# Leqr/MSMP-PDE

Hardware: AMD Instinct MI355X
Metric: rollout-steps/sec (whole node), E2 nx=100 tw=25 (higher is better)
Workload: dtype f32; 1 GPU; E2 MSMP-PDE (MP_PDE_SolverLEMLinGated), 2048 graphs x nx=100, time_window=25, 6 gated layer pairs, radius graph n=3; graphs_total=2048, graphs_per_gpu=2048, nodes_per_gpu=204800, edges_per_gpu=1204224, parallelism=dp1 (graph-sharded, no collective in the rollout), sub_batches=1, range_policy_switched_to_exact_fp32=False, preheat=170 untimed steps (>= 1 s) after the 5 warm-up steps

## Files before the change

### msmp-pde_amd/csrc/lem_kernel.hip

```cpp
#include "lem_layout.h"
#include <type_traits>

namespace msmp {

struct LemPackArgs {
    const float *w, *wz, *b, *bz, *wa, *ba, *wb, *bb;
    int ninp;
    float* out;
};

__global__ void pack_lem_kernel(LemPackArgs a) {
    const LemLayout L = lem_layout();
    const int kin = H + a.ninp;
    for (int64_t p = (int64_t)blockIdx.x * blockDim.x + threadIdx.x; p < L.scales; p += (int64_t)gridDim.x * blockDim.x) {
        float v = 0.f;
        if (p < L.mlp) {
            const int ch = (int)(p / CHUNK_FLOATS), row = (int)(p % CHUNK_FLOATS) / KC, kk = (int)(p % KC);
            const int grp = ch >> 2, k = (ch & 3) * KC + kk;
            if (grp == 0) v = a.w[(size_t)(H + row) * kin + k];
            else if (grp == 1) v = a.w[(size_t)(2 * H + row) * kin + k];
            else if (grp == 2) v = a.w[(size_t)row * kin + k];
            else v = a.wz[(size_t)row * kin + k];
        } else if (p < L.bias) {
            const int64_t o = p - L.mlp;
// ... 158 lines not shown
        for (int T = 0; T < 4; ++T)
#pragma unroll
            for (int r = 0; r < 16; ++r)
                z[T][0][r] = (1.0f - g[T][0][r]) * z[T][0][r] + g[T][0][r] * tanhf_(acc[T][0][r]);
        lem_acc_init<NS>(a, 0, lane, hh, x, g);
        LEM_GROUP(y, g, 8, a.rec + 12 * CHUNK_FLOATS)
#pragma unroll
        for (int T = 0; T < 4; ++T)
#pragma unroll
            for (int r = 0; r < 16; ++r) g[T][0][r] = a.dt * sigmoidf_(g[T][0][r]);
        lem_acc_init<NS>(a, 3, lane, hh, x, acc);
        LEM_GROUP(z, acc, 12, after)
#pragma unroll
        for (int T = 0; T < 4; ++T)
#pragma unroll
            for (int r = 0; r < 16; ++r)
                y[T][0][r] = (1.0f - g[T][0][r]) * y[T][0][r] + g[T][0][r] * tanhf_(acc[T][0][r]);
    }
#undef LEM_GROUP

    if (a.with_mlp) {
        acc_init_bias<1>(a.mlpb, hh, acc);
#pragma unroll
        for (int j = 0; j < 4; ++j) {
            wstage_load(ws, a.mlp + (size_t)(j + 1) * CHUNK_FLOATS, tid);
            mma_chunk_from_acc<1>(lds + (j & 1) * H * LDW, c, hh, y[j], acc);
            wstage_store(ws, lds + ((j + 1) & 1) * H * LDW, tid);
            __syncthreads();
        }
#pragma unroll
        for (int T = 0; T < 4; ++T)
#pragma unroll
            for (int r = 0; r < 16; ++r) acc[T][0][r] = swishf(acc[T][0][r]);
        acc_init_bias<1>(a.mlpb + H, hh, y);
#pragma unroll
        for (int j = 0; j < 4; ++j) {
            if (j < 3) wstage_load(ws, a.mlp + (size_t)(4 + j + 1) * CHUNK_FLOATS, tid);
            mma_chunk_from_acc<1>(lds + (j & 1) * H * LDW, c, hh, acc[j], y);
            if (j < 3) {
                wstage_store(ws, lds + ((j + 1) & 1) * H * LDW, tid);
                __syncthreads();
            }
        }
#pragma unroll
        for (int T = 0; T < 4; ++T)
#pragma unroll
            for (int r = 0; r < 16; ++r) y[T][0][r] = swishf(y[T][0][r]);
    }

    if (n < a.n_nodes) {
        float* o = a.out + (size_t)n * H + 4 * hh;
#pragma unroll
        for (int T = 0; T < 4; ++T)
#pragma unroll
            for (int q = 0; q < 4; ++q) {
                f32x4 v;
#pragma unroll
                for (int m = 0; m < 4; ++m) v[m] = y[T][0][4 * q + m];
                *reinterpret_cast<f32x4*>(o + 32 * T + 8 * q) = v;
            }
    }
}


struct LemWsArgs {
    const float* xin;
    const float* u;
    const float* pos_x;
    const float* pos_t;
    const float* vars;
    const float* dt_cum;
    int tw, nv;
    long n_nodes;
    int t_len, with_mlp;
    float dt;
    const float* rec_s;
    const float* mlp_s;
    const float* bias_s;
    const float* wx_h;
    const float* mlpb_s;
    const float* scales;
    float* out;
    int full_wgs = 0x7fffffff;
};

constexpr int LEM_WS_FR = 1024;

template <int P, int MODE>
__device__ __forceinline__ void lem_ws_load_x(const LemWsArgs& a, const float* xc, long node, int t, float (&x)[2 * ((P + 1) / 2)]) {
    constexpr int NS = (P + 1) / 2;
    if (MODE == 0) {
        const f32x2* p = reinterpret_cast<const f32x2*>(a.xin + ((size_t)node * a.t_len + t) * (2 * NS));
#pragma unroll
        for (int i = 0; i < NS; ++i) {
            const f32x2 v = p[i];
            x[2 * i] = v[0];
            x[2 * i + 1] = v[1];
        }
    } else {
#pragma unroll
        for (int i = 0; i < NS; ++i) {
            const f32x2 v = *reinterpret_cast<const f32x2*>(xc + 2 * i);
            x[2 * i] = v[0];
            x[2 * i + 1] = v[1];
        }
        if (MODE == 1) {
            x[1] = a.u[(size_t)node * a.tw + t];
        } else {
            x[1] = a.u[(size_t)node * 2 * a.tw + t];
            x[2] = a.u[(size_t)node * 2 * a.tw + a.tw + t];
            x[3] = a.dt_cum[t] + x[3];
        }
    }
}

template <int P>
__device__ __forceinline__ void lem_ws_slots(const float (&x)[2 * ((P + 1) / 2)], int hh, half8 (&bx)[(3 * P + 2 + 15) / 16]) {
    constexpr int M = (3 * P + 2 + 15) / 16;
    _Float16 xh[P], xl[P];
#pragma unroll
    for (int f = 0; f < P; ++f) {
        xh[f] = (_Float16)x[f];
        xl[f] = (_Float16)(x[f] - (float)xh[f]);
    }
#pragma unroll
    for (int m = 0; m < M; ++m)
#pragma unroll
        for (int j = 0; j < 8; ++j) {
            const int s0 = 16 * m + j, s1 = 16 * m + 8 + j;
            const _Float16 v0 = s0 < 3 * P ? (s0 / P == 1 ? xl[s0 % P] : xh[s0 % P]) : (_Float16)(s0 < 3 * P + 2 ? 1.f : 0.f);
            const _Float16 v1 = s1 < 3 * P ? (s1 / P == 1 ? xl[s1 % P] : xh[s1 % P]) : (_Float16)(s1 < 3 * P + 2 ? 1.f : 0.f);
            bx[m][j] = hh ? v1 : v0;
        }
}

template <int P, int MODE>
__device__ __forceinline__ void lem_ws3_patch(const float (&xd)[MODE == 1 ? 1 : 3], int hh, half8 (&bx)[(3 * P + 2 + 15) / 16]) {
    constexpr int ND = MODE == 1 ? 1 : 3;
#pragma unroll
    for (int k = 0; k < ND; ++k) {
        const int f = 1 + k;
        const _Float16 h = (_Float16)xd[k];
        const _Float16 l = (_Float16)(xd[k] - (float)h);
#pragma unroll
        for (int p = 0; p < 3; ++p) {
            const int s = p * P + f, m = s >> 4, hhs = (s >> 3) & 1, j = s & 7;
            bx[m][j] = hh == hhs ? (p == 1 ? l : h) : bx[m][j];
        }
    }
}

__device__ __forceinline__ void lem_ws_bias(const float* bl, int hh, f32x16& acc) {
#pragma unroll
    for (int q = 0; q < 4; ++q) {
        const f32x4 bv = *reinterpret_cast<const f32x4*>(bl + 8 * q + 4 * hh);
#pragma unroll
        for (int m = 0; m < 4; ++m) acc[4 * q + m] = bv[m];
    }
}

__device__ __forceinline__ void lem_ws_publish(const f32x16& st, half8* area, int ks, int lane) {
#pragma unroll
    for (int s = 0; s < 2; ++s) {
        float v[8];
#pragma unroll
        for (int j = 0; j < 8; ++j) v[j] = st[8 * s + j];
        half8 hi, lo;
        split8(v, hi, lo);
        area[((ks * 2 + s) * 2 + 0) * 64 + lane] = hi;
        area[((ks * 2 + s) * 2 + 1) * 64 + lane] = lo;
    }
}

__device__ __forceinline__ float vmin(float a, float b) {
    float d;
    asm("v_min_f32 %0, %1, %2" : "=v"(d) : "v"(a), "v"(b));
    return d;
}

__device__ __forceinline__ void lem_ws_update_publish_q(const f32x16& a0, const f32x16& a1, float c0, float c1, float idt, f32x16& st,
                                                        half8* area, int ks, int lane) {
#pragma unroll
    for (int s = 0; s < 2; ++s) {
        half8 phi, plo;
#pragma unroll
        for (int i = 0; i < 8; i += 2) {
            f32x2 sv;
#pragma unroll
            for (int e = 0; e < 2; ++e) {
                const int r = 8 * s + i + e;
                const float ea = msmp_exp2(a0[r] * c0);
                const float eb = msmp_exp2(vmin(a1[r] * c1, 60.f));
                const float qb = eb + 1.0f;
                const float rr = msmp_rcp(__builtin_fmaf(ea, idt, idt) * qb);
                sv[e] = __builtin_fmaf(rr, __builtin_fmaf(-st[r], qb, 1.0f - eb), st[r]);
                st[r] = sv[e];
            }
            const half2 hp = __builtin_convertvector(sv, half2);
            const half2 lp = split_lo_pair(hp, sv);
            phi[i] = hp[0];
            phi[i + 1] = hp[1];
            plo[i] = lp[0];
            plo[i + 1] = lp[1];
        }
        area[((ks * 2 + s) * 2 + 0) * 64 + lane] = phi;
        area[((ks * 2 + s) * 2 + 1) * 64 + lane] = plo;
    }
}

constexpr int LEM_SCHED_NOT_MFMA = 0x7F6;

#if MSMP_PROF_LEM
__device__ unsigned long long g_prof_lem[16];
#define LPROF_DECL unsigned lp_m = 0, lp_v = 0, lp_b = 0, lp_w = 0, lp_t = (unsigned)__builtin_readcyclecounter();
#define LPROF(var) do { const unsigned t_ = (unsigned)__builtin_readcyclecounter(); var += t_ - lp_t; lp_t = t_; } while (0)
#define LPROF_FLUSH if (lane == 0 && ks == 0 && (blockIdx.x & 31) == 0) { unsigned long long* o = g_prof_lem + 4 * role; atomicAdd(o, (unsigned long long)lp_m); atomicAdd(o + 1, (unsigned long long)lp_v); atomicAdd(o + 2, (unsigned long long)lp_b); atomicAdd(o + 3, 1ull); atomicAdd(g_prof_lem + 8 + role, (unsigned long long)lp_w); }
#else
#define LPROF_DECL unsigned lp_w = 0; (void)lp_w;
#define LPROF(var)
#define LPROF_FLUSH
#endif
#define LEM_SYNC() do { LPROF(lp_w); __syncthreads(); LPROF(lp_b); } while (0)

template <bool SAME, int OFF0, int OFF1>
__device__ __forceinline__ void lem_ws3_gemm2(const half8 (&w0)[4][2][2], const half8 (&w1)[4][2][2], const char* b0, const char* b1,
                                              f32x16& acc0, f32x16& acc1) {
    if (!SAME) {
        constexpr int FB = 64 * 16;
        auto frag = [&](int n, int plane) -> half8 {
            const int f = (n >> 1) * 2 + plane;
            return (n & 1) ? *reinterpret_cast<const half8*>(b1 + OFF1 + f * FB) : *reinterpret_cast<const half8*>(b0 + OFF0 + f * FB);
        };
        half8 h = frag(0, 0), l = frag(0, 1);
#pragma unroll
        for (int n = 0; n < 16; ++n) {
            const int kt = n >> 2, s = (n >> 1) & 1;
            half8 hn = h, ln = l;
            if (n < 15) hn = frag(n + 1, 0);
            __builtin_amdgcn_sched_barrier(0);
            if (n & 1) {
                acc1 = __builtin_amdgcn_mfma_f32_32x32x16_f16(w1[kt][s][1], h, acc1, 0, 0, 0);
                acc1 = __builtin_amdgcn_mfma_f32_32x32x16_f16(w1[kt][s][0], l, acc1, 0, 0, 0);
            } else {
                acc0 = __builtin_amdgcn_mfma_f32_32x32x16_f16(w0[kt][s][1], h, acc0, 0, 0, 0);
                acc0 = __builtin_amdgcn_mfma_f32_32x32x16_f16(w0[kt][s][0], l, acc0, 0, 0, 0);
            }
            __builtin_amdgcn_sched_barrier(0);
            if (n < 15) ln = frag(n + 1, 1);
            __builtin_amdgcn_sched_barrier(0);
            if (n & 1) acc1 = __builtin_amdgcn_mfma_f32_32x32x16_f16(w1[kt][s][0], h, acc1, 0, 0, 0);
            else acc0 = __builtin_amdgcn_mfma_f32_32x32x16_f16(w0[kt][s][0], h, acc0, 0, 0, 0);
            __builtin_amdgcn_sched_barrier(0);
            h = hn;
            l = ln;
        }
        return;
    }
#pragma unroll
    for (int kt = 0; kt < 4; ++kt)
#pragma unroll
        for (int s = 0; s < 2; ++s) {
            constexpr int FB = 64 * 16;
            const int f = (kt * 2 + s) * 2;
            const half8 h0 = *reinterpret_cast<const half8*>(b0 + OFF0 + f * FB), l0 = *reinterpret_cast<const half8*>(b0 + OFF0 + (f + 1) * FB);
            half8 h1 = h0, l1 = l0;
            if (!SAME) {
                h1 = *reinterpret_cast<const half8*>(b1 + OFF1 + f * FB);
                l1 = *reinterpret_cast<const half8*>(b1 + OFF1 + (f + 1) * FB);
            }
            MSMP_MFMA_LOLO(2, acc0, w0[kt][s][1], l0);
            MSMP_MFMA_LOLO(2, acc1, w1[kt][s][1], l1);
            acc0 = __builtin_amdgcn_mfma_f32_32x32x16_f16(w0[kt][s][1], h0, acc0, 0, 0, 0);
            acc0 = __builtin_amdgcn_mfma_f32_32x32x16_f16(w0[kt][s][0], l0, acc0, 0, 0, 0);
            acc0 = __builtin_amdgcn_mfma_f32_32x32x16_f16(w0[kt][s][0], h0, acc0, 0, 0, 0);
            __builtin_amdgcn_sched_barrier(LEM_SCHED_NOT_MFMA);
            acc1 = __builtin_amdgcn_mfma_f32_32x32x16_f16(w1[kt][s][1], h1, acc1, 0, 0, 0);
            acc1 = __builtin_amdgcn_mfma_f32_32x32x16_f16(w1[kt][s][0], l1, acc1, 0, 0, 0);
            acc1 = __builtin_amdgcn_mfma_f32_32x32x16_f16(w1[kt][s][0], h1, acc1, 0, 0, 0);
            __builtin_amdgcn_sched_barrier(LEM_SCHED_NOT_MFMA);
        }
}

template <int P, int MODE>
__global__ __launch_bounds__(512) void lem_encoder_ws3_kernel(LemWsArgs a) {
    constexpr int NS = (P + 1) / 2, M = (3 * P + 2 + 15) / 16;
    __shared__ __attribute__((aligned(16))) float lds[6 * SPLIT_CHUNK_FLOATS + 768];
    __shared__ __attribute__((aligned(16))) float xconst[96 * 8];
    __shared__ half8 bxc[3 * M * 64];
    __shared__ half8 wxl[8 * 2 * M * 64];
    half8* const yfr = reinterpret_cast<half8*>(lds);
    half8* const zfr = yfr + 3 * LEM_WS_FR;
    float* const bias_l = lds + 6 * SPLIT_CHUNK_FLOATS;
    const int tid = threadIdx.x, lane = tid & 63;
    const int wave = __builtin_amdgcn_readfirstlane(tid >> 6);
    const int ks = wave & 3, role = wave >> 2;
    const int c = lane & 31, hh = lane >> 5;
    const bool single = (int)blockIdx.x >= a.full_wgs;
    const long n0 = single ? 96L * a.full_wgs + 32L * ((int)blockIdx.x - a.full_wgs) : (long)blockIdx.x * 96;
    const long n_lim = single ? (n0 + 32 < a.n_nodes ? n0 + 32 : a.n_nodes) : a.n_nodes;
    const int nt = single ? 1 : 3;
    const float LOG2E = 1.44269504088896340736f;
    const float inv_w = a.scales[4], inv_z = a.scales[5];
    const int T = a.t_len;

    {
        half8 zero;
#pragma unroll
        for (int j = 0; j < 8; ++j) zero[j] = (_Float16)0.f;
#pragma unroll
        for (int i = 0; i < 6; ++i) yfr[tid + 512 * i] = zero;
        bias_l[tid] = a.bias_s[tid];
        if (tid < 256) bias_l[512 + tid] = a.mlpb_s[tid];
        if (MODE != 0 && tid < 96) {
            const long nn = n0 + tid < a.n_nodes ? n0 + tid : a.n_nodes - 1;
            float* row = xconst + 8 * tid;
#pragma unroll
            for (int f = 0; f < 8; ++f) row[f] = 0.f;
            row[0] = a.pos_x[nn];
            if (MODE == 1) {
                for (int f = 0; f < a.nv; ++f) row[2 + f] = a.vars[(size_t)nn * a.nv + f];
            } else {
                row[3] = a.pos_t[nn];
                for (int f = 1; f < a.nv; ++f) row[3 + f] = a.vars[(size_t)nn * a.nv + f];
            }
        }
    }
    half8 w[2][4][2][2];
    half8* const wxw = wxl + (size_t)wave * (2 * M * 64) + lane;
    {
        const half8* rs = reinterpret_cast<const half8*>(a.rec_s);
        const half8* wh = reinterpret_cast<const half8*>(a.wx_h);
#pragma unroll
        for (int gi = 0; gi < 2; ++gi) {
            const int grp = 2 * role + gi;
#pragma unroll
            for (int kt = 0; kt < 4; ++kt)
#pragma unroll
                for (int s = 0; s < 2; ++s)
#pragma unroll
                    for (int pl = 0; pl < 2; ++pl)
                        w[gi][kt][s][pl] = rs[(size_t)(grp * 4 + kt) * 1024 + ((s * 4 + ks) * 2 + pl) * 64 + lane];
#pragma unroll
            for (int m = 0; m < M; ++m) wxw[(gi * M + m) * 64] = wh[((grp * 4 + ks) * 2 + m) * 64 + lane];
        }
    }
    const float c0 = -inv_w * LOG2E, c1 = -2.0f * (role ? inv_z : inv_w) * LOG2E, idt = 1.0f / a.dt;

    f32x16 st[3];
#pragma unroll
    for (int X = 0; X < 3; ++X)
#pragma unroll
        for (int r = 0; r < 16; ++r) st[X][r] = 0.f;
    constexpr int ZBASE = 3 * LEM_WS_FR * 16;
    const char* lb_y;
    const char* lb_z;
    {
        unsigned lo = lane * 16;
        asm volatile("" : "+v"(lo));
        lb_y = reinterpret_cast<const char*>(lds) + lo;
        unsigned lo2 = lane * 16 + ZBASE;
        asm volatile("" : "+v"(lo2));
        lb_z = reinterpret_cast<const char*>(lds) + lo2;
    }
    float xn[2 * NS];
    f32x16 acc0, acc1;
#pragma unroll
    for (int r = 0; r < 16; ++r) { acc0[r] = 0.f; acc1[r] = 0.f; }
    __syncthreads();

    float xd[MODE == 1 ? 1 : 3];
    if (MODE != 0 && tid < 192) {
        const int Xt = tid >> 6, l64 = tid & 63;
        float xs[2 * NS];
#pragma unroll
        for (int f = 0; f < 2 * NS; ++f) xs[f] = xconst[8 * (32 * Xt + (l64 & 31)) + f];
        if (MODE == 2) xs[3] = 0.f;
        half8 b0[M];
        lem_ws_slots<P>(xs, l64 >> 5, b0);
#pragma unroll
        for (int m = 0; m < M; ++m) bxc[(Xt * M + m) * 64 + l64] = b0[m];
    }
    __syncthreads();
    auto fetch_x = [&](auto Xc, int t) {
        constexpr int X = decltype(Xc)::value;
        const long n = n0 + 32 * X + c;
        if (MODE != 0) {
            const long node = n < a.n_nodes ? n : a.n_nodes - 1;
            if (MODE == 1) {
                xd[0] = a.u[(size_t)node * a.tw + t];
            } else {
                xd[0] = a.u[(size_t)node * 2 * a.tw + t];
                xd[MODE == 1 ? 0 : 1] = a.u[(size_t)node * 2 * a.tw + a.tw + t];
                xd[MODE == 1 ? 0 : 2] = a.dt_cum[t] + xconst[8 * (32 * X + c) + 3];
            }
            return;
        }
        lem_ws_load_x<P, MODE>(a, xconst + 8 * (32 * X + c), n < a.n_nodes ? n : a.n_nodes - 1, t, xn);
    };
    auto half_m = [&](auto Xc) {
        constexpr int X = decltype(Xc)::value;
        half8 bx[M];
        __builtin_amdgcn_sched_barrier(0);
        if (MODE != 0) {
#pragma unroll
            for (int m = 0; m < M; ++m) bx[m] = bxc[(X * M + m) * 64 + lane];
            lem_ws3_patch<P, MODE>(xd, hh, bx);
        } else {
            lem_ws_slots<P>(xn, hh, bx);
        }
        const f32x16 zero = {0.f, 0.f, 0.f, 0.f, 0.f, 0.f, 0.f, 0.f, 0.f, 0.f, 0.f, 0.f, 0.f, 0.f, 0.f, 0.f};
        acc0 = __builtin_amdgcn_mfma_f32_32x32x16_f16(wxw[0], bx[0], zero, 0, 0, 0);
        acc1 = __builtin_amdgcn_mfma_f32_32x32x16_f16(wxw[M * 64], bx[0], zero, 0, 0, 0);
#pragma unroll
        for (int m = 1; m < M; ++m) {
            acc0 = __builtin_amdgcn_mfma_f32_32x32x16_f16(wxw[m * 64], bx[m], acc0, 0, 0, 0);
            acc1 = __builtin_amdgcn_mfma_f32_32x32x16_f16(wxw[(M + m) * 64], bx[m], acc1, 0, 0, 0);
        }
        constexpr int YO = X * LEM_WS_FR * 16, ZO = (3 + X) * LEM_WS_FR * 16 - ZBASE;
        if (role) lem_ws3_gemm2<false, YO, ZO>(w[0], w[1], lb_y, lb_z, acc0, acc1);
        else lem_ws3_gemm2<true, YO, YO>(w[0], w[1], lb_y, lb_y, acc0, acc1);
    };
    auto half_v = [&](auto Xc) {
        constexpr int X = decltype(Xc)::value;
        lem_ws_update_publish_q(acc0, acc1, c0, c1, idt, st[X], (role ? yfr : zfr) + X * LEM_WS_FR, ks, lane);
    };
    using I0 = std::integral_constant<int, 0>;
    using I1 = std::integral_constant<int, 1>;
    using I2 = std::integral_constant<int, 2>;

    LPROF_DECL
    if (single) {
        if (!role) {
            fetch_x(I0{}, 0);
            for (int t = 0; t < T; ++t) {
                { half_m(I0{}); LPROF(lp_m); }                                                   LEM_SYNC();
                fetch_x(I0{}, t + 1 < T ? t + 1 : t); { half_v(I0{}); LPROF(lp_v); }             LEM_SYNC();
                LEM_SYNC();
                LEM_SYNC();
            }
        } else {
            for (int t = 0; t < T; ++t) {
                LEM_SYNC();
                fetch_x(I0{}, t);                                                               LEM_SYNC();
                { half_m(I0{}); LPROF(lp_m); }                                                   LEM_SYNC();
                { half_v(I0{}); LPROF(lp_v); }                                                   LEM_SYNC();
            }
        }
    } else
    if (!role) {
        fetch_x(I0{}, 0);
        for (int t = 0; t < T; ++t) {
            { half_m(I0{}); LPROF(lp_m); }                                           LEM_SYNC();
            fetch_x(I1{}, t); { half_v(I0{}); LPROF(lp_v); }                         LEM_SYNC();
            { half_m(I1{}); LPROF(lp_m); }                                           LEM_SYNC();
            fetch_x(I2{}, t); { half_v(I1{}); LPROF(lp_v); }                         LEM_SYNC();
            { half_m(I2{}); LPROF(lp_m); }                                           LEM_SYNC();
            fetch_x(I0{}, t + 1 < T ? t + 1 : t); { half_v(I2{}); LPROF(lp_v); }     LEM_SYNC();
        }
        LEM_SYNC();
        LEM_SYNC();
        LEM_SYNC();
    } else {
        LEM_SYNC();
        LEM_SYNC();
        fetch_x(I0{}, 0);                                           LEM_SYNC();
        { half_m(I0{}); LPROF(lp_m); }                                               LEM_SYNC();
        fetch_x(I1{}, 0); { half_v(I0{}); LPROF(lp_v); }                             LEM_SYNC();
        { half_m(I1{}); LPROF(lp_m); }                                               LEM_SYNC();
        for (int t = 1; t < T; ++t) {
            fetch_x(I2{}, t - 1); { half_v(I1{}); LPROF(lp_v); }                     LEM_SYNC();
            { half_m(I2{}); LPROF(lp_m); }                                           LEM_SYNC();
            fetch_x(I0{}, t); { half_v(I2{}); LPROF(lp_v); }                         LEM_SYNC();
            { half_m(I0{}); LPROF(lp_m); }                                           LEM_SYNC();
            fetch_x(I1{}, t); { half_v(I0{}); LPROF(lp_v); }                         LEM_SYNC();
            { half_m(I1{}); LPROF(lp_m); }                                           LEM_SYNC();
        }
        fetch_x(I2{}, T - 1); { half_v(I1{}); LPROF(lp_v); }                         LEM_SYNC();
        { half_m(I2{}); LPROF(lp_m); }                                               LEM_SYNC();
        { half_v(I2{}); LPROF(lp_v); }                                               LEM_SYNC();
    }
    LPROF_FLUSH

    if (a.with_mlp) {
        const half8* ms = reinterpret_cast<const half8*>(a.mlp_s);
#pragma unroll
        for (int gi = 0; gi < 2; ++gi)
#pragma unroll
            for (int kt = 0; kt < 4; ++kt)
#pragma unroll
                for (int s = 0; s < 2; ++s)
#pragma unroll
                    for (int pl = 0; pl < 2; ++pl)
                        w[gi][kt][s][pl] = ms[(size_t)(gi * 4 + kt) * 1024 + ((s * 4 + ks) * 2 + pl) * 64 + lane];
        const float invA = a.scales[6], invB = a.scales[7];
        for (int pass = 0; pass < 2; ++pass) {
            const int X = pass ? 2 : role;
            const bool work = (pass == 0 || role == 0) && X < nt;
            const half8* yb = yfr + X * LEM_WS_FR;
            half8* hb = zfr + X * LEM_WS_FR;
            if (work) {
                f32x16 acc;
                lem_ws_bias(bias_l + 512 + 32 * ks, hh, acc);
#pragma unroll
                for (int kt = 0; kt < 4; ++kt)
#pragma unroll
                    for (int s = 0; s < 2; ++s) {
                        const half8 h0 = yb[((kt * 2 + s) * 2 + 0) * 64 + lane], l0 = yb[((kt * 2 + s) * 2 + 1) * 64 + lane];
                        MSMP_MFMA_LOLO(2, acc, w[0][kt][s][1], l0);
                        acc = __builtin_amdgcn_mfma_f32_32x32x16_f16(w[0][kt][s][1], h0, acc, 0, 0, 0);
                        acc = __builtin_amdgcn_mfma_f32_32x32x16_f16(w[0][kt][s][0], l0, acc, 0, 0, 0);
                        acc = __builtin_amdgcn_mfma_f32_32x32x16_f16(w[0][kt][s][0], h0, acc, 0, 0, 0);
                    }
#pragma unroll
                for (int r = 0; r < 16; ++r) acc[r] = swishf(acc[r] * invA);
                lem_ws_publish(acc, hb, ks, lane);
            }
            __syncthreads();
            if (work) {
                f32x16 res;
                lem_ws_bias(bias_l + 512 + H + 32 * ks, hh, res);
#pragma unroll
                for (int kt = 0; kt < 4; ++kt)
#pragma unroll
                    for (int s = 0; s < 2; ++s) {
                        const half8 h0 = hb[((kt * 2 + s) * 2 + 0) * 64 + lane], l0 = hb[((kt * 2 + s) * 2 + 1) * 64 + lane];
                        MSMP_MFMA_LOLO(2, res, w[1][kt][s][1], l0);
                        res = __builtin_amdgcn_mfma_f32_32x32x16_f16(w[1][kt][s][1], h0, res, 0, 0, 0);
                        res = __builtin_amdgcn_mfma_f32_32x32x16_f16(w[1][kt][s][0], l0, res, 0, 0, 0);
                        res = __builtin_amdgcn_mfma_f32_32x32x16_f16(w[1][kt][s][0], h0, res, 0, 0, 0);
                    }
                const long n = n0 + 32 * X + c;
                if (n < n_lim) {
                    float* o = a.out + (size_t)n * H + 32 * ks + 4 * hh;
#pragma unroll
                    for (int q = 0; q < 4; ++q) {
                        f32x4 v;
#pragma unroll
                        for (int m = 0; m < 4; ++m) v[m] = swishf(res[4 * q + m] * invB);
                        *reinterpret_cast<f32x4*>(o + 8 * q) = v;
                    }
                }
            }
        }
    } else if (role) {
#pragma unroll
        for (int X = 0; X < 3; ++X) {
            const long n = n0 + 32 * X + c;
            if (n < n_lim) {
                float* o = a.out + (size_t)n * H + 32 * ks + 4 * hh;
#pragma unroll
                for (int q = 0; q < 4; ++q) {
                    f32x4 v;
#pragma unroll
                    for (int m = 0; m < 4; ++m) v[m] = st[X][4 * q + m];
                    *reinterpret_cast<f32x4*>(o + 8 * q) = v;
                }
            }
        }
    }
}

__global__ __launch_bounds__(256) void pack_lem_b3_kernel(const float* __restrict__ chunks, int n_chunks, float* __restrict__ out) {
    const int id = blockIdx.x * 256 + threadIdx.x;
    if (id >= n_chunks * 512) return;
    const int lane = id & 63, T = (id >> 6) & 3, s = (id >> 8) & 1, ch = id >> 9;
    const int m = lane & 31, hh = lane >> 5;
    float v[8];
#pragma unroll
    for (int j = 0; j < 8; ++j) v[j] = chunks[(size_t)ch * CHUNK_FLOATS + (32 * T + m) * KC + split_k_acc(s, hh, j)];
    const Bf3 f = split_bf16x3(v);
    u32x4* dst = reinterpret_cast<u32x4*>(out) + (size_t)ch * LEM_B3_CHUNK_U4 + (size_t)((s * 4 + T) * 3) * 64 + lane;
    dst[0] = __builtin_bit_cast(u32x4, f.hi);
    dst[64] = __builtin_bit_cast(u32x4, f.mid);
    dst[128] = __builtin_bit_cast(u32x4, f.lo);
}

}

using namespace msmp;

#if MSMP_PROF_LEM
extern "C" __attribute__((visibility("default"))) int msmp_debug_prof_lem(unsigned long long* out16, int reset) {
    if (reset) { unsigned long long z[16] = {0}; return (int)hipMemcpyToSymbol(HIP_SYMBOL(g_prof_lem), z, sizeof(z)); }
    return (int)hipMemcpyFromSymbol(out16, HIP_SYMBOL(g_prof_lem), 16 * sizeof(unsigned long long));
}
#endif
static unsigned lem_partition_for(int64_t n_nodes, int cus, int tail, int* full_wgs) {
    const int64_t tiles = (n_nodes + 31) / 32, groups = (n_nodes + 95) / 96;
    *full_wgs = 0x7fffffff;
    if (!tail || cus < 1) return (unsigned)groups;
    const int64_t full = (groups / cus) * cus;
    const int64_t rem = tiles - 3 * full;
    if (rem <= 0) return (unsigned)groups;
    const double all_three = (double)((groups + cus - 1) / cus), mixed = (double)(full / cus) + 0.5 * (double)((rem + cus - 1) / cus);
    if (mixed > all_three - 0.3) return (unsigned)groups;
    *full_wgs = (int)full;
    return (unsigned)(full + rem);
}
static unsigned lem_partition(int64_t n_nodes, int* full_wgs) {
    int dev = 0, cus = 0;
    if (hipGetDevice(&dev) != hipSuccess || hipDeviceGetAttribute(&cus, hipDeviceAttributeMultiprocessorCount, dev) != hipSuccess || cus <= 0) cus = 256;
    cus = cus / msmp_tune_get("lem_share");
    if (cus < 1) cus = 1;
    return lem_partition_for(n_nodes, cus, msmp_tune_get("lem_tail"), full_wgs);
}
extern "C" __attribute__((visibility("default"))) int msmp_debug_lem_partition(int64_t n_nodes, int cus, int64_t* grid_out, int64_t* full_out) {
    int full = 0;
    const unsigned g = lem_partition_for(n_nodes, cus, 1, &full);
    if (grid_out) *grid_out = g;
    if (full_out) *full_out = full == 0x7fffffff ? (int64_t)g : full;
    return 0;
}
extern "C" int64_t msmp_packed_lem_floats(void) { return lem_layout().total; }

extern "C" int msmp_pack_lem_f32(const float* weights, const float* weights_lin_z, const float* bias, const float* bias_lin_z,
                                 const float* mlp_w0, const float* mlp_b0, const float* mlp_w1, const float* mlp_b1,
                                 int ninp, float* packed_out, msmp_stream_t stream) {
    MSMP_REQUIRE(weights && weights_lin_z && bias && bias_lin_z && packed_out, MSMP_ERR_ARG, "msmp_pack_lem_f32: null pointer");
    MSMP_REQUIRE(ninp >= 1 && ninp <= LEM_MAX_INP, MSMP_ERR_UNSUPPORTED, "msmp_pack_lem_f32: ninp=%d outside 1..%d", ninp, LEM_MAX_INP);
    const bool mlp = mlp_w0 && mlp_b0 && mlp_w1 && mlp_b1;
    MSMP_REQUIRE(mlp || !(mlp_w0 || mlp_b0 || mlp_w1 || mlp_b1), MSMP_ERR_ARG, "msmp_pack_lem_f32: give all four mlp tensors or none");
    LemPackArgs a{weights, weights_lin_z, bias, bias_lin_z, mlp_w0, mlp_b0, mlp_w1, mlp_b1, ninp, packed_out};
    hipLaunchKernelGGL(pack_lem_kernel, dim3(256), dim3(256), 0, (hipStream_t)stream, a);
    hipLaunchKernelGGL(pack_lem_scale_kernel, dim3(4), dim3(256), 0, (hipStream_t)stream, a);
    hipLaunchKernelGGL(pack_lem_split_kernel, dim3(256), dim3(256), 0, (hipStream_t)stream, a);
    hipLaunchKernelGGL(pack_lem_b3_kernel, dim3(16 * 512 / 256), dim3(256), 0, (hipStream_t)stream, packed_out + lem_layout().rec, 16,
                       packed_out + lem_layout().rec_b3);
    return check_launch("pack_lem_kernel");
}

extern "C" int msmp_lem_input_stride(int ninp) { return ninp >= 1 && ninp <= LEM_MAX_INP ? 2 * ((ninp + 1) / 2) : -1; }

static LemWsArgs lem_ws_args(const float* packed, int64_t n_nodes, int t_len, int with_mlp, float dt, float* h_out) {
    const LemLayout L = lem_layout();
    LemWsArgs a{};
    a.n_nodes = (long)n_nodes;
    a.t_len = t_len;
    a.with_mlp = with_mlp;
    a.dt = dt;
    a.rec_s = packed + L.rec_s;
    a.mlp_s = packed + L.mlp_s;
    a.bias_s = packed + L.bias_s;
    a.wx_h = packed + L.wx_h;
    a.mlpb_s = packed + L.mlpb_s;
    a.scales = packed + L.scales;
    a.out = h_out;
    return a;
}

template <int MODE, int P = MODE == 0 ? 1 : MODE + 2>
static void lem_ws3_launch(LemWsArgs a, int ninp, hipStream_t st) {
    if constexpr (P < 8)
        if (ninp != P) return lem_ws3_launch<MODE, P + 1>(a, ninp, st);
    const unsigned grid = lem_partition(a.n_nodes, &a.full_wgs);
    hipLaunchKernelGGL((lem_encoder_ws3_kernel<P, MODE>), dim3(grid), dim3(512), 0, st, a);
}

extern "C" int msmp_lem_encoder_f32(const float* xin, int64_t n_nodes, int t_len, int ninp, float dt, const float* packed,
                                    int with_mlp, float* h_out, msmp_stream_t stream) {
    MSMP_REQUIRE(xin && packed && h_out, MSMP_ERR_ARG, "msmp_lem_encoder_f32: null pointer");
    MSMP_REQUIRE(n_nodes > 0 && n_nodes < (1L << 31) && t_len >= 1, MSMP_ERR_ARG, "msmp_lem_encoder_f32: bad sizes");
    MSMP_REQUIRE(ninp >= 1 && ninp <= LEM_MAX_INP, MSMP_ERR_UNSUPPORTED, "msmp_lem_encoder_f32: ninp=%d outside 1..%d", ninp, LEM_MAX_INP);
    const bool split = msmp_tune_get("split") != 0;
    hipStream_t st = (hipStream_t)stream;
    timing_begin(MSMP_K_LEM, st);
    if (split) {
        LemWsArgs wa = lem_ws_args(packed, n_nodes, t_len, with_mlp, dt, h_out);
        wa.xin = xin;
        lem_ws3_launch<0>(wa, ninp, st);
    } else {
        const LemLayout L = lem_layout();
        LemArgs a{xin, (long)n_nodes, t_len, with_mlp, dt, packed + L.rec, packed + L.mlp, packed + L.bias, packed + L.wx,
                  packed + L.mlpb, h_out};
        const unsigned grid = (unsigned)((n_nodes + 127) / 128);
        switch ((ninp + 1) / 2) {
            case 1: hipLaunchKernelGGL(lem_encoder_kernel<1>, dim3(grid), dim3(256), 0, st, a); break;
            case 2: hipLaunchKernelGGL(lem_encoder_kernel<2>, dim3(grid), dim3(256), 0, st, a); break;
            case 3: hipLaunchKernelGGL(lem_encoder_kernel<3>, dim3(grid), dim3(256), 0, st, a); break;
            default: hipLaunchKernelGGL(lem_encoder_kernel<4>, dim3(grid), dim3(256), 0, st, a); break;
        }
    }
    timing_end(MSMP_K_LEM, st);
    return check_launch(split ? "lem_encoder_ws3_kernel" : "lem_encoder_kernel");
}

extern "C" int msmp_lem_encoder_nodes_f32(const float* u, const float* pos_x, const float* pos_t, const float* vars, const float* dt_cum,
                                          int64_t n_nodes, int tw, int nv, int two_d, float dt, const float* packed, int with_mlp,
                                          float* h_out, msmp_stream_t stream) {
    MSMP_REQUIRE(u && pos_x && vars && packed && h_out, MSMP_ERR_ARG, "msmp_lem_encoder_nodes_f32: null pointer");
    MSMP_REQUIRE(!two_d || (pos_t && dt_cum), MSMP_ERR_ARG, "msmp_lem_encoder_nodes_f32: the 2-D input needs pos_t and dt_cum");
    MSMP_REQUIRE(n_nodes > 0 && n_nodes < (1L << 31) && tw >= 1 && nv >= 1, MSMP_ERR_ARG, "msmp_lem_encoder_nodes_f32: bad sizes");
    const int ninp = (two_d ? 3 : 2) + nv;
    MSMP_REQUIRE(ninp <= LEM_MAX_INP, MSMP_ERR_UNSUPPORTED, "msmp_lem_encoder_nodes_f32: ninp=%d > %d", ninp, LEM_MAX_INP);
    MSMP_REQUIRE(msmp_tune_get("split"), MSMP_ERR_UNSUPPORTED, "msmp_lem_encoder_nodes_f32: only on the fp16-split path (weight-stationary kernel)");
    LemWsArgs wa = lem_ws_args(packed, n_nodes, tw, with_mlp, dt, h_out);
    wa.u = u;
    wa.pos_x = pos_x;
    wa.pos_t = pos_t;
    wa.vars = vars;
    wa.dt_cum = dt_cum;
    wa.tw = tw;
    wa.nv = nv;
    hipStream_t st = (hipStream_t)stream;
    timing_begin(MSMP_K_LEM, st);
    if (two_d) lem_ws3_launch<2>(wa, ninp, st);
    else lem_ws3_launch<1>(wa, ninp, st);
    timing_end(MSMP_K_LEM, st);
    return check_launch("lem_encoder_ws3_kernel");
}
```

Measured before the change: 164.4 rollout-steps/s.

## Make LEM encoder persistent over work items and overlap MLP epilogue with recurrence drain

Turns the warp-specialised LEM encoder into a persistent kernel. The grid is capped at the CU count and each workgroup walks work items, so weights and biases are loaded once per workgroup instead of once per tile. The MLP epilogue is interleaved into the drain barriers of the recurrence roles, with MLP weights streamed per group. The first LDS fragments are prefetched before the input-projection MFMAs, and the same-input gemm path is software-pipelined. The cost is more complex barrier accounting, guarded by a static_assert, and possibly reduced occupancy or parallelism when there are fewer items than CUs.

```diff
diff --git a/msmp-pde_amd/csrc/lem_kernel.hip b/msmp-pde_amd/csrc/lem_kernel.hip
--- a/msmp-pde_amd/csrc/lem_kernel.hip
+++ b/msmp-pde_amd/csrc/lem_kernel.hip
@@ -264,7 +264,30 @@
     const float* scales;
     float* out;
     int full_wgs = 0x7fffffff;
+    int n_items = 0;
 };
+
+__host__ __device__ inline long lem_item_first_node(long item, long full_wgs, int* nt) {
+    const bool single = item >= full_wgs;
+    *nt = single ? 1 : 3;
+    return single ? 96L * full_wgs + 32L * (item - full_wgs) : 96L * item;
+}
+
+constexpr int LEM_ITEM_PROLOGUE_BARRIERS = 2, LEM_FILL = 3, LEM_DRAIN = 3;
+constexpr int lem_barriers_a(int T, int nt, bool mlp) {
+    return LEM_ITEM_PROLOGUE_BARRIERS + (nt == 1 ? 4 * T : 6 * T + LEM_DRAIN) + (mlp ? 1 : 0);
+}
+constexpr int lem_barriers_b(int T, int nt, bool mlp) {
+    return LEM_ITEM_PROLOGUE_BARRIERS + (nt == 1 ? 4 * T : LEM_FILL + 3 + 6 * (T - 1) + 3) + (mlp ? 1 : 0);
+}
+constexpr bool lem_barriers_match() {
+    for (int T = 1; T <= 64; ++T)
+        for (int nt = 1; nt <= 3; nt += 2)
+            for (int mlp = 0; mlp < 2; ++mlp)
+                if (lem_barriers_a(T, nt, mlp != 0) != lem_barriers_b(T, nt, mlp != 0)) return false;
+    return true;
+}
+static_assert(lem_barriers_match(), "lem_encoder_ws3_kernel: the two roles must execute the same number of barriers per work item");
 
 constexpr int LEM_WS_FR = 1024;
 
@@ -394,31 +417,39 @@
 
 #if MSMP_PROF_LEM
 __device__ unsigned long long g_prof_lem[16];
-#define LPROF_DECL unsigned lp_m = 0, lp_v = 0, lp_b = 0, lp_w = 0, lp_t = (unsigned)__builtin_readcyclecounter();
+#define LPROF_DECL unsigned lp_m = 0, lp_v = 0, lp_b = 0, lp_w = 0, lp_p = 0, lp_e = 0, lp_t = (unsigned)__builtin_readcyclecounter();
 #define LPROF(var) do { const unsigned t_ = (unsigned)__builtin_readcyclecounter(); var += t_ - lp_t; lp_t = t_; } while (0)
-#define LPROF_FLUSH if (lane == 0 && ks == 0 && (blockIdx.x & 31) == 0) { unsigned long long* o = g_prof_lem + 4 * role; atomicAdd(o, (unsigned long long)lp_m); atomicAdd(o + 1, (unsigned long long)lp_v); atomicAdd(o + 2, (unsigned long long)lp_b); atomicAdd(o + 3, 1ull); atomicAdd(g_prof_lem + 8 + role, (unsigned long long)lp_w); }
+#define LPROF_FLUSH(n_done) if (lane == 0 && ks == 0 && (blockIdx.x & 31) == 0) { unsigned long long* o = g_prof_lem + 4 * role; atomicAdd(o, (unsigned long long)lp_m); atomicAdd(o + 1, (unsigned long long)lp_v); atomicAdd(o + 2, (unsigned long long)lp_b); atomicAdd(o + 3, (unsigned long long)(n_done)); atomicAdd(g_prof_lem + 8 + role, (unsigned long long)lp_w); atomicAdd(g_prof_lem + 10 + role, (unsigned long long)lp_p); atomicAdd(g_prof_lem + 12 + role, (unsigned long long)lp_e); }
 #else
 #define LPROF_DECL unsigned lp_w = 0; (void)lp_w;
 #define LPROF(var)
-#define LPROF_FLUSH
+#define LPROF_FLUSH(n_done)
 #endif
 #define LEM_SYNC() do { LPROF(lp_w); __syncthreads(); LPROF(lp_b); } while (0)
 
 template <bool SAME, int OFF0, int OFF1>
+__device__ __forceinline__ void lem_ws3_frag0(const char* b0, const char* b1, half8& h, half8& l, half8& hn) {
+    constexpr int FB = 64 * 16;
+    h = *reinterpret_cast<const half8*>(b0 + OFF0);
+    l = *reinterpret_cast<const half8*>(b0 + OFF0 + FB);
+    hn = SAME ? *reinterpret_cast<const half8*>(b0 + OFF0 + 2 * FB) : *reinterpret_cast<const half8*>(b1 + OFF1);
+}
+
+template <bool SAME, int OFF0, int OFF1>
 __device__ __forceinline__ void lem_ws3_gemm2(const half8 (&w0)[4][2][2], const half8 (&w1)[4][2][2], const char* b0, const char* b1,
-                                              f32x16& acc0, f32x16& acc1) {
+                                              f32x16& acc0, f32x16& acc1, half8 h, half8 l, half8 hn1) {
     if (!SAME) {
         constexpr int FB = 64 * 16;
         auto frag = [&](int n, int plane) -> half8 {
             const int f = (n >> 1) * 2 + plane;
             return (n & 1) ? *reinterpret_cast<const half8*>(b1 + OFF1 + f * FB) : *reinterpret_cast<const half8*>(b0 + OFF0 + f * FB);
         };
-        half8 h = frag(0, 0), l = frag(0, 1);
 #pragma unroll
         for (int n = 0; n < 16; ++n) {
             const int kt = n >> 2, s = (n >> 1) & 1;
             half8 hn = h, ln = l;
-            if (n < 15) hn = frag(n + 1, 0);
+            if (n == 0) hn = hn1;
+            else if (n < 15) hn = frag(n + 1, 0);
             __builtin_amdgcn_sched_barrier(0);
             if (n & 1) {
                 acc1 = __builtin_amdgcn_mfma_f32_32x32x16_f16(w1[kt][s][1], h, acc1, 0, 0, 0);
@@ -438,29 +469,26 @@
         }
         return;
     }
-#pragma unroll
-    for (int kt = 0; kt < 4; ++kt)
-#pragma unroll
-        for (int s = 0; s < 2; ++s) {
-            constexpr int FB = 64 * 16;
-            const int f = (kt * 2 + s) * 2;
-            const half8 h0 = *reinterpret_cast<const half8*>(b0 + OFF0 + f * FB), l0 = *reinterpret_cast<const half8*>(b0 + OFF0 + (f + 1) * FB);
-            half8 h1 = h0, l1 = l0;
-            if (!SAME) {
-                h1 = *reinterpret_cast<const half8*>(b1 + OFF1 + f * FB);
-                l1 = *reinterpret_cast<const half8*>(b1 + OFF1 + (f + 1) * FB);
-            }
-            MSMP_MFMA_LOLO(2, acc0, w0[kt][s][1], l0);
-            MSMP_MFMA_LOLO(2, acc1, w1[kt][s][1], l1);
-            acc0 = __builtin_amdgcn_mfma_f32_32x32x16_f16(w0[kt][s][1], h0, acc0, 0, 0, 0);
-            acc0 = __builtin_amdgcn_mfma_f32_32x32x16_f16(w0[kt][s][0], l0, acc0, 0, 0, 0);
-            acc0 = __builtin_amdgcn_mfma_f32_32x32x16_f16(w0[kt][s][0], h0, acc0, 0, 0, 0);
-            __builtin_amdgcn_sched_barrier(LEM_SCHED_NOT_MFMA);
-            acc1 = __builtin_amdgcn_mfma_f32_32x32x16_f16(w1[kt][s][1], h1, acc1, 0, 0, 0);
-            acc1 = __builtin_amdgcn_mfma_f32_32x32x16_f16(w1[kt][s][0], l1, acc1, 0, 0, 0);
-            acc1 = __builtin_amdgcn_mfma_f32_32x32x16_f16(w1[kt][s][0], h1, acc1, 0, 0, 0);
-            __builtin_amdgcn_sched_barrier(LEM_SCHED_NOT_MFMA);
-        }
+    constexpr int FB = 64 * 16;
+    half8 hn = hn1;
+#pragma unroll
+    for (int n = 0; n < 8; ++n) {
+        const int kt = n >> 1, s = n & 1;
+        __builtin_amdgcn_sched_barrier(0);
+        MSMP_MFMA_LOLO(2, acc0, w0[kt][s][1], l);
+        MSMP_MFMA_LOLO(2, acc1, w1[kt][s][1], l);
+        acc0 = __builtin_amdgcn_mfma_f32_32x32x16_f16(w0[kt][s][1], h, acc0, 0, 0, 0);
+        acc0 = __builtin_amdgcn_mfma_f32_32x32x16_f16(w0[kt][s][0], l, acc0, 0, 0, 0);
+        acc0 = __builtin_amdgcn_mfma_f32_32x32x16_f16(w0[kt][s][0], h, acc0, 0, 0, 0);
+        __builtin_amdgcn_sched_barrier(LEM_SCHED_NOT_MFMA);
+        acc1 = __builtin_amdgcn_mfma_f32_32x32x16_f16(w1[kt][s][1], h, acc1, 0, 0, 0);
+        acc1 = __builtin_amdgcn_mfma_f32_32x32x16_f16(w1[kt][s][0], l, acc1, 0, 0, 0);
+        acc1 = __builtin_amdgcn_mfma_f32_32x32x16_f16(w1[kt][s][0], h, acc1, 0, 0, 0);
+        __builtin_amdgcn_sched_barrier(0);
+        if (n < 7) l = *reinterpret_cast<const half8*>(b0 + OFF0 + (2 * n + 3) * FB);
+        h = hn;
+        if (n < 6) hn = *reinterpret_cast<const half8*>(b0 + OFF0 + (2 * n + 4) * FB);
+    }
 }
 
 template <int P, int MODE>
@@ -477,36 +505,16 @@
     const int wave = __builtin_amdgcn_readfirstlane(tid >> 6);
     const int ks = wave & 3, role = wave >> 2;
     const int c = lane & 31, hh = lane >> 5;
-    const bool single = (int)blockIdx.x >= a.full_wgs;
-    const long n0 = single ? 96L * a.full_wgs + 32L * ((int)blockIdx.x - a.full_wgs) : (long)blockIdx.x * 96;
-    const long n_lim = single ? (n0 + 32 < a.n_nodes ? n0 + 32 : a.n_nodes) : a.n_nodes;
-    const int nt = single ? 1 : 3;
+    LPROF_DECL
     const float LOG2E = 1.44269504088896340736f;
     const float inv_w = a.scales[4], inv_z = a.scales[5];
+    const float invA = a.scales[6], invB = a.scales[7];
     const int T = a.t_len;
-
-    {
-        half8 zero;
-#pragma unroll
-        for (int j = 0; j < 8; ++j) zero[j] = (_Float16)0.f;
-#pragma unroll
-        for (int i = 0; i < 6; ++i) yfr[tid + 512 * i] = zero;
-        bias_l[tid] = a.bias_s[tid];
-        if (tid < 256) bias_l[512 + tid] = a.mlpb_s[tid];
-        if (MODE != 0 && tid < 96) {
-            const long nn = n0 + tid < a.n_nodes ? n0 + tid : a.n_nodes - 1;
-            float* row = xconst + 8 * tid;
-#pragma unroll
-            for (int f = 0; f < 8; ++f) row[f] = 0.f;
-            row[0] = a.pos_x[nn];
-            if (MODE == 1) {
-                for (int f = 0; f < a.nv; ++f) row[2 + f] = a.vars[(size_t)nn * a.nv + f];
-            } else {
-                row[3] = a.pos_t[nn];
-                for (int f = 1; f < a.nv; ++f) row[3 + f] = a.vars[(size_t)nn * a.nv + f];
-            }
-        }
-    }
+    bool single = false;
+    long n0 = 0, n_lim = 0;
+
+    bias_l[tid] = a.bias_s[tid];
+    if (tid < 256) bias_l[512 + tid] = a.mlpb_s[tid];
     half8 w[2][4][2][2];
     half8* const wxw = wxl + (size_t)wave * (2 * M * 64) + lane;
     {
@@ -529,10 +537,6 @@
     const float c0 = -inv_w * LOG2E, c1 = -2.0f * (role ? inv_z : inv_w) * LOG2E, idt = 1.0f / a.dt;
 
     f32x16 st[3];
-#pragma unroll
-    for (int X = 0; X < 3; ++X)
-#pragma unroll
-        for (int r = 0; r < 16; ++r) st[X][r] = 0.f;
     constexpr int ZBASE = 3 * LEM_WS_FR * 16;
     const char* lb_y;
     const char* lb_z;
@@ -548,26 +552,13 @@
     f32x16 acc0, acc1;
 #pragma unroll
     for (int r = 0; r < 16; ++r) { acc0[r] = 0.f; acc1[r] = 0.f; }
-    __syncthreads();
 
     float xd[MODE == 1 ? 1 : 3];
-    if (MODE != 0 && tid < 192) {
-        const int Xt = tid >> 6, l64 = tid & 63;
-        float xs[2 * NS];
-#pragma unroll
-        for (int f = 0; f < 2 * NS; ++f) xs[f] = xconst[8 * (32 * Xt + (l64 & 31)) + f];
-        if (MODE == 2) xs[3] = 0.f;
-        half8 b0[M];
-        lem_ws_slots<P>(xs, l64 >> 5, b0);
-#pragma unroll
-        for (int m = 0; m < M; ++m) bxc[(Xt * M + m) * 64 + l64] = b0[m];
-    }
-    __syncthreads();
     auto fetch_x = [&](auto Xc, int t) {
         constexpr int X = decltype(Xc)::value;
-        const long n = n0 + 32 * X + c;
+        const unsigned n = (unsigned)n0 + 32u * X + (unsigned)c, n_last = (unsigned)a.n_nodes - 1u;
         if (MODE != 0) {
-            const long node = n < a.n_nodes ? n : a.n_nodes - 1;
+            const unsigned node = n < n_last ? n : n_last;
             if (MODE == 1) {
                 xd[0] = a.u[(size_t)node * a.tw + t];
             } else {
@@ -577,30 +568,33 @@
             }
             return;
         }
-        lem_ws_load_x<P, MODE>(a, xconst + 8 * (32 * X + c), n < a.n_nodes ? n : a.n_nodes - 1, t, xn);
+        lem_ws_load_x<P, MODE>(a, xconst + 8 * (32 * X + c), (long)(n < n_last ? n : n_last), t, xn);
     };
     auto half_m = [&](auto Xc) {
         constexpr int X = decltype(Xc)::value;
         half8 bx[M];
         __builtin_amdgcn_sched_barrier(0);
+        constexpr int YO = X * LEM_WS_FR * 16, ZO = (3 + X) * LEM_WS_FR * 16 - ZBASE;
         if (MODE != 0) {
 #pragma unroll
             for (int m = 0; m < M; ++m) bx[m] = bxc[(X * M + m) * 64 + lane];
-            lem_ws3_patch<P, MODE>(xd, hh, bx);
-        } else {
-            lem_ws_slots<P>(xn, hh, bx);
-        }
+        }
+        const half8 wa0 = wxw[0], wb0 = wxw[M * 64];
+        if (MODE != 0) lem_ws3_patch<P, MODE>(xd, hh, bx);
+        else lem_ws_slots<P>(xn, hh, bx);
         const f32x16 zero = {0.f, 0.f, 0.f, 0.f, 0.f, 0.f, 0.f, 0.f, 0.f, 0.f, 0.f, 0.f, 0.f, 0.f, 0.f, 0.f};
-        acc0 = __builtin_amdgcn_mfma_f32_32x32x16_f16(wxw[0], bx[0], zero, 0, 0, 0);
-        acc1 = __builtin_amdgcn_mfma_f32_32x32x16_f16(wxw[M * 64], bx[0], zero, 0, 0, 0);
+        acc0 = __builtin_amdgcn_mfma_f32_32x32x16_f16(wa0, bx[0], zero, 0, 0, 0);
+        acc1 = __builtin_amdgcn_mfma_f32_32x32x16_f16(wb0, bx[0], zero, 0, 0, 0);
 #pragma unroll
         for (int m = 1; m < M; ++m) {
             acc0 = __builtin_amdgcn_mfma_f32_32x32x16_f16(wxw[m * 64], bx[m], acc0, 0, 0, 0);
             acc1 = __builtin_amdgcn_mfma_f32_32x32x16_f16(wxw[(M + m) * 64], bx[m], acc1, 0, 0, 0);
         }
-        constexpr int YO = X * LEM_WS_FR * 16, ZO = (3 + X) * LEM_WS_FR * 16 - ZBASE;
-        if (role) lem_ws3_gemm2<false, YO, ZO>(w[0], w[1], lb_y, lb_z, acc0, acc1);
-        else lem_ws3_gemm2<true, YO, YO>(w[0], w[1], lb_y, lb_y, acc0, acc1);
+        half8 fh, fl, fhn;
+        if (role) lem_ws3_frag0<false, YO, ZO>(lb_y, lb_z, fh, fl, fhn);
+        else lem_ws3_frag0<true, YO, YO>(lb_y, lb_y, fh, fl, fhn);
+        if (role) lem_ws3_gemm2<false, YO, ZO>(w[0], w[1], lb_y, lb_z, acc0, acc1, fh, fl, fhn);
+        else lem_ws3_gemm2<true, YO, YO>(w[0], w[1], lb_y, lb_y, acc0, acc1, fh, fl, fhn);
     };
     auto half_v = [&](auto Xc) {
         constexpr int X = decltype(Xc)::value;
@@ -610,7 +604,120 @@
     using I1 = std::integral_constant<int, 1>;
     using I2 = std::integral_constant<int, 2>;
 
-    LPROF_DECL
+    auto opaque = [](int v) { asm volatile("" : "+v"(v)); return v; };
+    half8 mw[4][2][2];
+    auto mlp_load = [&](int gi) {
+        const unsigned lo = (unsigned)(ks * 128 + opaque(lane)) * 16u;
+        unsigned mo = (unsigned)gi * (4096u * 16u);
+        asm volatile("" : "+s"(mo));
+        const char* ms = reinterpret_cast<const char*>(a.mlp_s) + mo;
+#pragma unroll
+        for (int kt = 0; kt < 4; ++kt)
+#pragma unroll
+            for (int s = 0; s < 2; ++s)
+#pragma unroll
+                for (int pl = 0; pl < 2; ++pl)
+                    mw[kt][s][pl] = *reinterpret_cast<const half8*>(ms + (size_t)(kt * 1024 + (s * 8 + pl) * 64) * 16 + lo);
+    };
+    auto mlp_gemm = [&](const half8* in, f32x16& acc) {
+#pragma unroll
+        for (int kt = 0; kt < 4; ++kt)
+#pragma unroll
+            for (int s = 0; s < 2; ++s) {
+                const half8 h0 = in[((kt * 2 + s) * 2 + 0) * 64], l0 = in[((kt * 2 + s) * 2 + 1) * 64];
+                MSMP_MFMA_LOLO(2, acc, mw[kt][s][1], l0);
+                acc = __builtin_amdgcn_mfma_f32_32x32x16_f16(mw[kt][s][1], h0, acc, 0, 0, 0);
+                acc = __builtin_amdgcn_mfma_f32_32x32x16_f16(mw[kt][s][0], l0, acc, 0, 0, 0);
+                acc = __builtin_amdgcn_mfma_f32_32x32x16_f16(mw[kt][s][0], h0, acc, 0, 0, 0);
+            }
+    };
+    auto mlp_hidden = [&](int X) {
+        const int lq = opaque(lane);
+        f32x16 acc;
+        lem_ws_bias(bias_l + 512 + 32 * ks, lq >> 5, acc);
+        mlp_gemm(yfr + X * LEM_WS_FR + lq, acc);
+#pragma unroll
+        for (int r = 0; r < 16; ++r) acc[r] = swishf(acc[r] * invA);
+        lem_ws_publish(acc, zfr + X * LEM_WS_FR, ks, lq);
+    };
+    auto mlp_out = [&](int X) {
+        const int lq = opaque(lane);
+        f32x16 res;
+        lem_ws_bias(bias_l + 512 + H + 32 * ks, lq >> 5, res);
+        mlp_gemm(zfr + X * LEM_WS_FR + lq, res);
+        const long n = n0 + 32 * X + (lq & 31);
+        if (n < n_lim) {
+            float* o = a.out + (size_t)n * H + 32 * ks + 4 * (lq >> 5);
+#pragma unroll
+            for (int q = 0; q < 4; ++q) {
+                f32x4 v;
+#pragma unroll
+                for (int m = 0; m < 4; ++m) v[m] = swishf(res[4 * q + m] * invB);
+                *reinterpret_cast<f32x4*>(o + 8 * q) = v;
+            }
+        }
+    };
+    auto store_y = [&](auto Xc) {
+        constexpr int X = decltype(Xc)::value;
+        const int lq = opaque(lane);
+        const long n = n0 + 32 * X + (lq & 31);
+        if (n < n_lim) {
+            float* o = a.out + (size_t)n * H + 32 * ks + 4 * (lq >> 5);
+#pragma unroll
+            for (int q = 0; q < 4; ++q) {
+                f32x4 v;
+#pragma unroll
+                for (int m = 0; m < 4; ++m) v[m] = st[X][4 * q + m];
+                *reinterpret_cast<f32x4*>(o + 8 * q) = v;
+            }
+        }
+    };
+
+    int n_done = 0;
+    auto walk = [&]() __attribute__((always_inline)) {
+    for (int item = blockIdx.x; item < a.n_items; item += gridDim.x, ++n_done) {
+    {
+        int nt_;
+        n0 = lem_item_first_node(item, a.full_wgs, &nt_);
+        single = nt_ == 1;
+        n_lim = single ? (n0 + 32 < a.n_nodes ? n0 + 32 : a.n_nodes) : a.n_nodes;
+        const int tq = opaque(lane) + 64 * wave;
+        const unsigned z0 = (unsigned)opaque(0);
+        const half8 zero = __builtin_bit_cast(half8, u32x4{z0, z0, z0, z0});
+#pragma unroll
+        for (int i = 0; i < 6; ++i) yfr[tq + 512 * i] = zero;
+#pragma unroll
+        for (int X = 0; X < 3; ++X)
+#pragma unroll
+            for (int r = 0; r < 16; ++r) st[X][r] = 0.f;
+        if (MODE != 0 && tq < 96) {
+            const long nn = n0 + tq < a.n_nodes ? n0 + tq : a.n_nodes - 1;
+            float* row = xconst + 8 * tq;
+#pragma unroll
+            for (int f = 0; f < 8; ++f) row[f] = __builtin_bit_cast(float, z0);
+            row[0] = a.pos_x[nn];
+            if (MODE == 1) {
+                for (int f = 0; f < a.nv; ++f) row[2 + f] = a.vars[(size_t)nn * a.nv + f];
+            } else {
+                row[3] = a.pos_t[nn];
+                for (int f = 1; f < a.nv; ++f) row[3 + f] = a.vars[(size_t)nn * a.nv + f];
+            }
+        }
+        __syncthreads();
+        if (MODE != 0 && tq < 192) {
+            const int Xt = tq >> 6, l64 = tq & 63;
+            float xs[2 * NS];
+#pragma unroll
+            for (int f = 0; f < 2 * NS; ++f) xs[f] = xconst[8 * (32 * Xt + (l64 & 31)) + f];
+            if (MODE == 2) xs[3] = 0.f;
+            half8 b0[M];
+            lem_ws_slots<P>(xs, l64 >> 5, b0);
+#pragma unroll
+            for (int m = 0; m < M; ++m) bxc[(Xt * M + m) * 64 + l64] = b0[m];
+        }
+        __syncthreads();
+    }
+    LPROF(lp_p);
     if (single) {
         if (!role) {
             fetch_x(I0{}, 0);
@@ -620,6 +727,10 @@
                 LEM_SYNC();
                 LEM_SYNC();
             }
+            if (a.with_mlp) {
+                mlp_load(0); mlp_hidden(0); mlp_load(1); LPROF(lp_e);                            __syncthreads();
+                mlp_out(0); LPROF(lp_e);
+            }
         } else {
             for (int t = 0; t < T; ++t) {
                 LEM_SYNC();
@@ -627,6 +738,9 @@
                 { half_m(I0{}); LPROF(lp_m); }                                                   LEM_SYNC();
                 { half_v(I0{}); LPROF(lp_v); }                                                   LEM_SYNC();
             }
+            if (a.with_mlp) __syncthreads();
+            else store_y(I0{});
+            LPROF(lp_e);
         }
     } else
     if (!role) {
@@ -639,9 +753,17 @@
             { half_m(I2{}); LPROF(lp_m); }                                           LEM_SYNC();
             fetch_x(I0{}, t + 1 < T ? t + 1 : t); { half_v(I2{}); LPROF(lp_v); }     LEM_SYNC();
         }
-        LEM_SYNC();
-        LEM_SYNC();
-        LEM_SYNC();
+        if (a.with_mlp) {
+            mlp_load(0); mlp_hidden(0); mlp_load(1); LPROF(lp_e);                    LEM_SYNC();
+            mlp_out(0); mlp_load(0); mlp_hidden(1); mlp_load(1); LPROF(lp_e);        LEM_SYNC();
+            mlp_out(1); mlp_load(0); LPROF(lp_e);                                    LEM_SYNC();
+            mlp_hidden(2); mlp_load(1); LPROF(lp_e);                                 __syncthreads();
+            mlp_out(2); LPROF(lp_e);
+        } else {
+            LEM_SYNC();
+            LEM_SYNC();
+            LEM_SYNC();
+        }
     } else {
         LEM_SYNC();
         LEM_SYNC();
@@ -660,86 +782,20 @@
         fetch_x(I2{}, T - 1); { half_v(I1{}); LPROF(lp_v); }                         LEM_SYNC();
         { half_m(I2{}); LPROF(lp_m); }                                               LEM_SYNC();
         { half_v(I2{}); LPROF(lp_v); }                                               LEM_SYNC();
-    }
-    LPROF_FLUSH
-
-    if (a.with_mlp) {
-        const half8* ms = reinterpret_cast<const half8*>(a.mlp_s);
-#pragma unroll
-        for (int gi = 0; gi < 2; ++gi)
-#pragma unroll
-            for (int kt = 0; kt < 4; ++kt)
-#pragma unroll
-                for (int s = 0; s < 2; ++s)
-#pragma unroll
-                    for (int pl = 0; pl < 2; ++pl)
-                        w[gi][kt][s][pl] = ms[(size_t)(gi * 4 + kt) * 1024 + ((s * 4 + ks) * 2 + pl) * 64 + lane];
-        const float invA = a.scales[6], invB = a.scales[7];
-        for (int pass = 0; pass < 2; ++pass) {
-            const int X = pass ? 2 : role;
-            const bool work = (pass == 0 || role == 0) && X < nt;
-            const half8* yb = yfr + X * LEM_WS_FR;
-            half8* hb = zfr + X * LEM_WS_FR;
-            if (work) {
-                f32x16 acc;
-                lem_ws_bias(bias_l + 512 + 32 * ks, hh, acc);
-#pragma unroll
-                for (int kt = 0; kt < 4; ++kt)
-#pragma unroll
-                    for (int s = 0; s < 2; ++s) {
-                        const half8 h0 = yb[((kt * 2 + s) * 2 + 0) * 64 + lane], l0 = yb[((kt * 2 + s) * 2 + 1) * 64 + lane];
-                        MSMP_MFMA_LOLO(2, acc, w[0][kt][s][1], l0);
-                        acc = __builtin_amdgcn_mfma_f32_32x32x16_f16(w[0][kt][s][1], h0, acc, 0, 0, 0);
-                        acc = __builtin_amdgcn_mfma_f32_32x32x16_f16(w[0][kt][s][0], l0, acc, 0, 0, 0);
-                        acc = __builtin_amdgcn_mfma_f32_32x32x16_f16(w[0][kt][s][0], h0, acc, 0, 0, 0);
-                    }
-#pragma unroll
-                for (int r = 0; r < 16; ++r) acc[r] = swishf(acc[r] * invA);
-                lem_ws_publish(acc, hb, ks, lane);
-            }
+        if (a.with_mlp) {
             __syncthreads();
-            if (work) {
-                f32x16 res;
-                lem_ws_bias(bias_l + 512 + H + 32 * ks, hh, res);
-#pragma unroll
-                for (int kt = 0; kt < 4; ++kt)
-#pragma unroll
-                    for (int s = 0; s < 2; ++s) {
-                        const half8 h0 = hb[((kt * 2 + s) * 2 + 0) * 64 + lane], l0 = hb[((kt * 2 + s) * 2 + 1) * 64 + lane];
-                        MSMP_MFMA_LOLO(2, res, w[1][kt][s][1], l0);
-                        res = __builtin_amdgcn_mfma_f32_32x32x16_f16(w[1][kt][s][1], h0, res, 0, 0, 0);
-                        res = __builtin_amdgcn_mfma_f32_32x32x16_f16(w[1][kt][s][0], l0, res, 0, 0, 0);
-                        res = __builtin_amdgcn_mfma_f32_32x32x16_f16(w[1][kt][s][0], h0, res, 0, 0, 0);
-                    }
-                const long n = n0 + 32 * X + c;
-                if (n < n_lim) {
-                    float* o = a.out + (size_t)n * H + 32 * ks + 4 * hh;
-#pragma unroll
-                    for (int q = 0; q < 4; ++q) {
-                        f32x4 v;
-#pragma unroll
-                        for (int m = 0; m < 4; ++m) v[m] = swishf(res[4 * q + m] * invB);
-                        *reinterpret_cast<f32x4*>(o + 8 * q) = v;
-                    }
-                }
-            }
-        }
-    } else if (role) {
-#pragma unroll
-        for (int X = 0; X < 3; ++X) {
-            const long n = n0 + 32 * X + c;
-            if (n < n_lim) {
-                float* o = a.out + (size_t)n * H + 32 * ks + 4 * hh;
-#pragma unroll
-                for (int q = 0; q < 4; ++q) {
-                    f32x4 v;
-#pragma unroll
-                    for (int m = 0; m < 4; ++m) v[m] = st[X][4 * q + m];
-                    *reinterpret_cast<f32x4*>(o + 8 * q) = v;
-                }
-            }
-        }
-    }
+        } else {
+            store_y(I0{});
+            store_y(I1{});
+            store_y(I2{});
+        }
+        LPROF(lp_e);
+    }
+    }
+    };
+    if (!role) walk();
+    else walk();
+    LPROF_FLUSH(n_done)
 }
 
 __global__ __launch_bounds__(256) void pack_lem_b3_kernel(const float* __restrict__ chunks, int n_chunks, float* __restrict__ out) {
@@ -779,12 +835,37 @@
     *full_wgs = (int)full;
     return (unsigned)(full + rem);
 }
-static unsigned lem_partition(int64_t n_nodes, int* full_wgs) {
+static unsigned lem_walk_grid(unsigned items, int cus) { return items < (unsigned)cus ? items : (unsigned)cus; }
+static int g_lem_cus_override = 0;
+static unsigned lem_partition(int64_t n_nodes, int* full_wgs, unsigned* grid) {
     int dev = 0, cus = 0;
     if (hipGetDevice(&dev) != hipSuccess || hipDeviceGetAttribute(&cus, hipDeviceAttributeMultiprocessorCount, dev) != hipSuccess || cus <= 0) cus = 256;
     cus = cus / msmp_tune_get("lem_share");
+    if (g_lem_cus_override > 0) cus = g_lem_cus_override;
     if (cus < 1) cus = 1;
-    return lem_partition_for(n_nodes, cus, msmp_tune_get("lem_tail"), full_wgs);
+    const unsigned items = lem_partition_for(n_nodes, cus, msmp_tune_get("lem_tail"), full_wgs);
+    *grid = lem_walk_grid(items, cus);
+    return items;
+}
+extern "C" __attribute__((visibility("default"))) int msmp_debug_lem_cus(int cus) {
+    const int before = g_lem_cus_override;
+    g_lem_cus_override = cus > 0 ? cus : 0;
+    return before;
+}
+extern "C" __attribute__((visibility("default"))) int msmp_debug_lem_walk(int64_t n_nodes, int cus, int64_t w, int64_t k, int64_t* first_out,
+                                                                            int64_t* count_out, int64_t* grid_out) {
+    int full = 0, nt = 0;
+    if (cus < 1) cus = 1;
+    const unsigned items = lem_partition_for(n_nodes, cus, 1, &full);
+    const unsigned grid = lem_walk_grid(items, cus);
+    if (grid_out) *grid_out = grid;
+    const int64_t item = w + k * (int64_t)grid;
+    if (w < 0 || k < 0 || w >= (int64_t)grid || item >= (int64_t)items) return 0;
+    const long n0 = lem_item_first_node((long)item, full, &nt);
+    const int64_t end = n0 + 32L * nt < n_nodes ? n0 + 32L * nt : n_nodes;
+    if (first_out) *first_out = n0;
+    if (count_out) *count_out = end > n0 ? end - n0 : 0;
+    return 1;
 }
 extern "C" __attribute__((visibility("default"))) int msmp_debug_lem_partition(int64_t n_nodes, int cus, int64_t* grid_out, int64_t* full_out) {
     int full = 0;
@@ -834,7 +915,8 @@
 static void lem_ws3_launch(LemWsArgs a, int ninp, hipStream_t st) {
     if constexpr (P < 8)
         if (ninp != P) return lem_ws3_launch<MODE, P + 1>(a, ninp, st);
-    const unsigned grid = lem_partition(a.n_nodes, &a.full_wgs);
+    unsigned grid = 0;
+    a.n_items = (int)lem_partition(a.n_nodes, &a.full_wgs, &grid);
     hipLaunchKernelGGL((lem_encoder_ws3_kernel<P, MODE>), dim3(grid), dim3(512), 0, st, a);
 }
 
```

New measurement: 166.4 rollout-steps/s, median of 6. 1.2% higher.
